# appyjain21/pilottai

Measured on AMD Instinct MI355X. Metric: completed agent-tasks/sec (whole node) + p50 task latency, 64 concurrent workers, higher is better.
Workload: dtype bf16

## Files before the change

### csrc/ops/attention.hip

```cpp
#include "common.h"

#include <algorithm>
#include <cstdlib>

namespace pa {

constexpr int ATT_HD = 128;
constexpr int ATT_BLK = 16;
constexpr int ATT_PART = 512;
constexpr float NEG_BIG = -1.0e30f;

template <int NW>
constexpr int att_lds_decode_bytes() { return (NW * 16 * (ATT_HD + 4) + 2 * NW * 16) * 4; }
constexpr int ATT_LDS_DECODE_BYTES = att_lds_decode_bytes<4>();
typedef __attribute__((address_space(1))) unsigned long long gu64;
typedef __attribute__((address_space(1))) int gi32;

__device__ __forceinline__ void att_store8(bf16* p, const bf16x8 v) { *reinterpret_cast<bf16x8*>(p) = v; }

template <int G, int NW = 4>
__device__ __forceinline__ void decode_item(
    const int4 it, char* smem, bf16* __restrict__ out, float* __restrict__ part_o,
    float* __restrict__ part_ml, int* __restrict__ counters, const bf16* __restrict__ q, const bf16* __restrict__ k_cache,
    const bf16* __restrict__ v_cache, const int* __restrict__ q_start, const int* __restrict__ q_len,
    const int* __restrict__ ctx_len, const int* __restrict__ block_table, int max_blocks, int H,
    int KV, int kvh, float scale_log2, int psz, int acq) {
  const int s = it.x, qb = it.y;
  const int nq = it.z & 0xff, part = (it.z >> 8) & 0xfff, nparts = it.z >> 20;
  const int pidx = it.w;
  const int lane = threadIdx.x & 63, wid = threadIdx.x >> 6;
  const int g = lane >> 4, col = lane & 15;
  const int hg = col % G, tq = col / G;
  const int ctx = ctx_len[s], ql = q_len[s], q0 = q_start[s];

  const bool colvalid = tq < nq;
  const int tok = qb + tq;
  const int key_limit = colvalid ? (ctx - ql + tok + 1) : 0;
  const int head = kvh * G + hg;
  const int causal_end = ctx - ql + qb + nq;
  const int kv_begin = nparts > 1 ? part * psz : 0;
  const int kv_end = nparts > 1 ? min(causal_end, kv_begin + psz) : causal_end;
  const int t_first = kv_begin >> 5;
  const int t_last = (kv_end + 31) >> 5;

  bf16x8 qf[4];
  {
    const bf16* qrow = q + ((size_t)(q0 + (colvalid ? tok : 0)) * H + head) * ATT_HD + 8 * g;
#pragma unroll
    for (int m = 0; m < 4; ++m) {
      bf16x8 v = *reinterpret_cast<const bf16x8*>(qrow + 32 * m);
      if (!colvalid) {
#pragma unroll
        for (int j = 0; j < 8; ++j) v[j] = (bf16)0.f;
      }
      qf[m] = v;
    }
  }

  const int* bt = block_table + (size_t)s * max_blocks;
  const int nblk = (ctx + ATT_BLK - 1) / ATT_BLK;
  const int kin = 8 * (col >> 2) + (col & 3);
  const size_t kv_stride_blk = (size_t)KV * ATT_BLK * ATT_HD;

  f32x4 o[8];
#pragma unroll
  for (int n = 0; n < 8; ++n) o[n] = f32x4{0.f, 0.f, 0.f, 0.f};
  float m_run = NEG_BIG, l_run = 0.f;

  auto load_tile = [&](int t, bf16x8 (&kf)[2][4], bf16x8 (&vf)[8]) {
    const int b0 = min(2 * t, nblk - 1), b1 = min(2 * t + 1, nblk - 1);
    const int pb0 = bt[b0], pb1 = bt[b1];
    const int pk = (kin >= 16) ? pb1 : pb0;
    const bf16* kbase = k_cache + (size_t)pk * kv_stride_blk +
                        (((size_t)kvh * 16 + g) * ATT_BLK + (kin & 15)) * 8;
#pragma unroll
    for (int c = 0; c < 2; ++c)
#pragma unroll
      for (int m = 0; m < 4; ++m)
        kf[c][m] = *reinterpret_cast<const bf16x8*>(kbase + (4 * m * ATT_BLK + 4 * c) * 8);
    const int pv = (g >> 1) ? pb1 : pb0;
    const bf16* vbase =
        v_cache + (size_t)pv * kv_stride_blk + ((size_t)kvh * ATT_HD + col) * ATT_BLK + 8 * (g & 1);
#pragma unroll
    for (int n = 0; n < 8; ++n)
      vf[n] = *reinterpret_cast<const bf16x8*>(vbase + (size_t)16 * n * ATT_BLK);
  };
  bf16x8 kf[2][4], vf[8];
  if (t_first + wid < t_last) load_tile(t_first + wid, kf, vf);
  for (int t = t_first + wid; t < t_last; t += NW) {
    bf16x8 kn[2][4], vn[8];
    if (t + NW < t_last) load_tile(t + NW, kn, vn);

    f32x4 sc[2];
#pragma unroll
    for (int c = 0; c < 2; ++c) {
      f32x4 acc = {0.f, 0.f, 0.f, 0.f};
#pragma unroll
      for (int m = 0; m < 4; ++m)
        acc = __builtin_amdgcn_mfma_f32_16x16x32_bf16(kf[c][m], qf[m], acc, 0, 0, 0);
      sc[c] = acc;
    }
    float tmax = NEG_BIG;
    const int kb = 32 * t + 8 * g;
#pragma unroll
    for (int c = 0; c < 2; ++c)
#pragma unroll
      for (int r = 0; r < 4; ++r) {
        const int key = kb + 4 * c + r;
        float v = sc[c][r] * scale_log2;
        v = (key < key_limit && key >= kv_begin) ? v : NEG_BIG;
        sc[c][r] = v;
        tmax = fmaxf(tmax, v);
      }
    tmax = fmaxf(tmax, __shfl_xor(tmax, 16, 64));
    tmax = fmaxf(tmax, __shfl_xor(tmax, 32, 64));
    const float m_new = fmaxf(m_run, tmax);
    const float alpha = exp2f(m_run - m_new);
    m_run = m_new;
    bf16x8 pf;
    float psum = 0.f;
#pragma unroll
    for (int c = 0; c < 2; ++c)
#pragma unroll
      for (int r = 0; r < 4; ++r) {
        const float p = exp2f(sc[c][r] - m_new);
        psum += p;
        pf[4 * c + r] = (bf16)p;
      }
    l_run = l_run * alpha + psum;
#pragma unroll
    for (int n = 0; n < 8; ++n) {
      o[n] *= alpha;
      o[n] = __builtin_amdgcn_mfma_f32_16x16x32_bf16(vf[n], pf, o[n], 0, 0, 0);
    }
#pragma unroll
    for (int c = 0; c < 2; ++c)
#pragma unroll
      for (int m = 0; m < 4; ++m) kf[c][m] = kn[c][m];
#pragma unroll
    for (int n = 0; n < 8; ++n) vf[n] = vn[n];
  }
  l_run += __shfl_xor(l_run, 16, 64);
  l_run += __shfl_xor(l_run, 32, 64);

  float(*lds_o)[16][ATT_HD + 4] = reinterpret_cast<float(*)[16][ATT_HD + 4]>(smem);
  float(*lds_m)[16] = reinterpret_cast<float(*)[16]>(smem + NW * 16 * (ATT_HD + 4) * sizeof(float));
  float(*lds_l)[16] = lds_m + NW;
#pragma unroll
  for (int n = 0; n < 8; ++n)
#pragma unroll
    for (int r = 0; r < 4; ++r) lds_o[wid][col][16 * n + 4 * g + r] = o[n][r];
  if (g == 0) {
    lds_m[wid][col] = m_run;
    lds_l[wid][col] = l_run;
  }
  __syncthreads();
  const bool mthr = NW == 4 || threadIdx.x < 256;
  const int ccol = (threadIdx.x >> 4) & 15;
  const int d0 = (threadIdx.x & 15) * 8;
  float mt = NEG_BIG;
#pragma unroll
  for (int w = 0; w < NW; ++w) mt = fmaxf(mt, lds_m[w][ccol]);
  float wgt[NW], L = 0.f;
#pragma unroll
  for (int w = 0; w < NW; ++w) {
    wgt[w] = exp2f(lds_m[w][ccol] - mt);
    L += wgt[w] * lds_l[w][ccol];
  }
  float acc[8];
#pragma unroll
  for (int j = 0; j < 8; ++j) {
    float a = 0.f;
#pragma unroll
    for (int w = 0; w < NW; ++w) a += wgt[w] * lds_o[w][ccol][d0 + j];
    acc[j] = a;
  }
  const int ctq = ccol / G, chg = ccol % G;
  if (nparts > 1) {
    const __amdgpu_buffer_rsrc_t ps = __builtin_amdgcn_make_buffer_rsrc(
        part_o + ((size_t)pidx * KV + kvh) * 16 * ATT_HD, 0, 16 * ATT_HD * 4, 0x00020000);
    const int soff = (ccol * ATT_HD + d0) * 4;
    if (mthr) {
      __builtin_amdgcn_raw_buffer_store_b128(__builtin_bit_cast(u32x4, f32x4{acc[0], acc[1], acc[2], acc[3]}),
                                             ps, soff, 0, 16);
      __builtin_amdgcn_raw_buffer_store_b128(__builtin_bit_cast(u32x4, f32x4{acc[4], acc[5], acc[6], acc[7]}),
                                             ps, soff + 16, 0, 16);
    }
    if (mthr && (threadIdx.x & 15) == 0) {
      const unsigned long long mlv =
          ((unsigned long long)__float_as_uint(L) << 32) | (unsigned long long)__float_as_uint(mt);
      __hip_atomic_store((gu64*)(part_ml + (((size_t)pidx * KV + kvh) * 16 + ccol) * 2), mlv,
                         __ATOMIC_RELAXED, __HIP_MEMORY_SCOPE_AGENT);
    }
    int* lflag = reinterpret_cast<int*>(smem + att_lds_decode_bytes<NW>());
    asm volatile("s_waitcnt vmcnt(0)" ::: "memory");
    if (!handoff_last(counters + (size_t)s * KV + kvh, nparts, lflag, acq) || ctq >= nq || !mthr) return;
    const int p0 = pidx - part;
    const __amdgpu_buffer_rsrc_t rs = __builtin_amdgcn_make_buffer_rsrc(
        part_o + (size_t)p0 * KV * 16 * ATT_HD, 0, nparts * KV * 16 * ATT_HD * 4, 0x00020000);
    auto load_ml = [&](int p) {
      return __hip_atomic_load((gu64*)(part_ml + (((size_t)(p0 + p) * KV + kvh) * 16 + ccol) * 2),
                               __ATOMIC_RELAXED, __HIP_MEMORY_SCOPE_AGENT);
    };
    float gm = NEG_BIG;
    for (int p = 0; p < nparts; ++p) gm = fmaxf(gm, __uint_as_float((unsigned)load_ml(p)));
    float GL = 0.f, ga[8] = {0.f, 0.f, 0.f, 0.f, 0.f, 0.f, 0.f, 0.f};
    for (int p = 0; p < nparts; ++p) {
      const unsigned long long v = load_ml(p);
      const float pmv = __uint_as_float((unsigned)v), plv = __uint_as_float((unsigned)(v >> 32));
      const float w = exp2f(pmv - gm);
      GL += w * plv;
      const int roff = (((p * KV + kvh) * 16 + ccol) * ATT_HD + d0) * 4;
      const f32x4 a = __builtin_bit_cast(f32x4, __builtin_amdgcn_raw_buffer_load_b128(rs, roff, 0, 16));
      const f32x4 b = __builtin_bit_cast(f32x4, __builtin_amdgcn_raw_buffer_load_b128(rs, roff + 16, 0, 16));
#pragma unroll
      for (int j = 0; j < 4; ++j) {
        ga[j] += w * a[j];
        ga[4 + j] += w * b[j];
      }
    }
    const float ginv = 1.f / GL;
    bf16x8 g8;
#pragma unroll
    for (int j = 0; j < 8; ++j) g8[j] = (bf16)(ga[j] * ginv);
    att_store8(out + ((size_t)(q0 + qb + ctq) * H + kvh * G + chg) * ATT_HD + d0, g8);
    return;
  }
  if (ctq >= nq || !mthr) return;
  const float inv = 1.f / L;
  bf16x8 w8;
#pragma unroll
  for (int j = 0; j < 8; ++j) w8[j] = (bf16)(acc[j] * inv);
  att_store8(out + ((size_t)(q0 + qb + ctq) * H + kvh * G + chg) * ATT_HD + d0, w8);
}

__device__ __forceinline__ int swap23(int x) { return (x & ~12) | ((x & 4) << 1) | ((x & 8) >> 1); }
constexpr int PF_LD = ATT_HD + 4;

__device__ __forceinline__ void softmax_pv_tile(f32x16 s, bool mask, int key0, int key_limit, float scale_log2,
                                                float& m_run, float& l_run, f32x16 (&o)[4],
                                                const bf16x8 (&vf)[2][4]) {
  if (mask) {
    const int lim = key_limit - key0;
#pragma unroll
    for (int g = 0; g < 16; ++g) s[g] = (16 * (g >> 3) + (g & 7)) < lim ? s[g] : NEG_BIG;
  }
  float tmax = s[0];
#pragma unroll
  for (int g = 1; g < 16; ++g) tmax = fmaxf(tmax, s[g]);
  tmax = fmaxf(tmax, __shfl_xor(tmax, 32, 64));
  const float m_new = fmaxf(m_run, tmax * scale_log2);
  if (__any(m_new > m_run)) {
    const float alpha = __builtin_amdgcn_exp2f(m_run - m_new);
    l_run *= alpha;
#pragma unroll
    for (int m = 0; m < 4; ++m) o[m] *= alpha;
    m_run = m_new;
  }
  const float nm = -m_run;
  float psum = 0.f;
  bf16x8 pf[2];
#pragma unroll
  for (int g = 0; g < 16; ++g) {
    const float p = __builtin_amdgcn_exp2f(fmaf(s[g], scale_log2, nm));
    psum += p;
    pf[g >> 3][g & 7] = (bf16)p;
  }
  l_run += psum;
#pragma unroll
  for (int st = 0; st < 2; ++st)
#pragma unroll
    for (int m = 0; m < 4; ++m) o[m] = __builtin_amdgcn_mfma_f32_32x32x16_bf16(vf[st][m], pf[st], o[m], 0, 0, 0);
}

__device__ __forceinline__ f32x16 qk_tile(const bf16x8 (&kf)[8], const bf16x8 (&qf)[8]) {
  f32x16 s;
#pragma unroll
  for (int j = 0; j < 16; ++j) s[j] = 0.f;
#pragma unroll
  for (int i = 0; i < 8; ++i) s = __builtin_amdgcn_mfma_f32_32x32x16_bf16(kf[i], qf[i], s, 0, 0, 0);
  return s;
}

template <int G, int NW = 4>
__device__ __forceinline__ void prefill_item(
    const int4 it, char* smem, bf16* __restrict__ out, const bf16* __restrict__ q,
    const bf16* __restrict__ k_cache, const bf16* __restrict__ v_cache,
    const int* __restrict__ q_start, const int* __restrict__ q_len, const int* __restrict__ ctx_len,
    const int* __restrict__ block_table, int max_blocks, int H, int KV, int kvh, float scale_log2) {
  const int s = it.x, qb = it.y, nq = it.z & 0xff;
  const int lane = threadIdx.x & 63, wid = threadIdx.x >> 6;
  const int r = lane & 31, h = lane >> 5;
  const int hg = r % G, tq = r / G;
  const int ctx = ctx_len[s], ql = q_len[s], q0 = q_start[s];
  const bool colvalid = tq < nq;
  const int tok = qb + tq;
  const int key_limit = colvalid ? (ctx - ql + tok + 1) : 0;
  const int head = kvh * G + hg;
  const int ntiles = (ctx - ql + qb + nq + 31) >> 5;
  const int kmin = ctx - ql + qb + 1;

  bf16x8 qf[8];
  {
    const bf16* qrow = q + ((size_t)(q0 + (colvalid ? tok : 0)) * H + head) * ATT_HD + 8 * h;
#pragma unroll
    for (int i = 0; i < 8; ++i) {
      bf16x8 v = *reinterpret_cast<const bf16x8*>(qrow + 16 * i);
      if (!colvalid) {
#pragma unroll
        for (int j = 0; j < 8; ++j) v[j] = (bf16)0.f;
      }
      qf[i] = v;
    }
  }
  const int* bt = block_table + (size_t)s * max_blocks;
  const int nblk = (ctx + ATT_BLK - 1) / ATT_BLK;
  const size_t kv_stride_blk = (size_t)KV * ATT_BLK * ATT_HD;
  const int krow = swap23(r);

  f32x16 o[4];
#pragma unroll
  for (int m = 0; m < 4; ++m)
#pragma unroll
    for (int j = 0; j < 16; ++j) o[m][j] = 0.f;
  float m_run = NEG_BIG, l_run = 0.f;

  for (int t = wid; t < ntiles; t += NW) {
    const int pb0 = bt[min(2 * t, nblk - 1)], pb1 = bt[min(2 * t + 1, nblk - 1)];
    const bf16* kbase = k_cache + (size_t)(krow >= 16 ? pb1 : pb0) * kv_stride_blk +
                        (((size_t)kvh * 16 + h) * ATT_BLK + (krow & 15)) * 8;
    bf16x8 kf[8];
#pragma unroll
    for (int i = 0; i < 8; ++i) kf[i] = *reinterpret_cast<const bf16x8*>(kbase + (size_t)2 * i * ATT_BLK * 8);
    bf16x8 vf[2][4];
#pragma unroll
    for (int st = 0; st < 2; ++st) {
      const bf16* vbase = v_cache + (size_t)(st ? pb1 : pb0) * kv_stride_blk +
                          ((size_t)kvh * ATT_HD + r) * ATT_BLK + 8 * h;
#pragma unroll
      for (int m = 0; m < 4; ++m) vf[st][m] = *reinterpret_cast<const bf16x8*>(vbase + (size_t)32 * m * ATT_BLK);
    }
    const f32x16 sc = qk_tile(kf, qf);
    softmax_pv_tile(sc, 32 * t + 32 > kmin, 32 * t + 8 * h, key_limit, scale_log2, m_run, l_run, o, vf);
  }
  l_run += __shfl_xor(l_run, 32, 64);

  float* lo = reinterpret_cast<float*>(smem);
  float* lm = lo + NW * 32 * PF_LD;
  float* ll = lm + NW * 32;
#pragma unroll
  for (int m = 0; m < 4; ++m)
#pragma unroll
    for (int gq = 0; gq < 4; ++gq) {
      f32x4 v = {o[m][4 * gq], o[m][4 * gq + 1], o[m][4 * gq + 2], o[m][4 * gq + 3]};
      *reinterpret_cast<f32x4*>(lo + (wid * 32 + r) * PF_LD + 32 * m + 8 * gq + 4 * h) = v;
    }
  if (h == 0) {
    lm[wid * 32 + r] = m_run;
    ll[wid * 32 + r] = l_run;
  }
  __syncthreads();
  const int ccol = threadIdx.x >> 3, d0 = (threadIdx.x & 7) * 16;
  const int ctq = ccol / G, chg = ccol % G;
  if (ctq >= nq || (NW == 8 && threadIdx.x >= 256)) return;
  float mt = NEG_BIG;
#pragma unroll
  for (int w = 0; w < NW; ++w) mt = fmaxf(mt, lm[w * 32 + ccol]);
  float wgt[NW], L = 0.f;
#pragma unroll
  for (int w = 0; w < NW; ++w) {
    wgt[w] = exp2f(lm[w * 32 + ccol] - mt);
    L += wgt[w] * ll[w * 32 + ccol];
  }
  const float inv = 1.f / L;
  bf16* orow = out + ((size_t)(q0 + qb + ctq) * H + kvh * G + chg) * ATT_HD + d0;
#pragma unroll
  for (int c8 = 0; c8 < 2; ++c8) {
    float acc[8] = {0.f, 0.f, 0.f, 0.f, 0.f, 0.f, 0.f, 0.f};
#pragma unroll
    for (int w = 0; w < NW; ++w) {
      const f32x4* src = reinterpret_cast<const f32x4*>(lo + (w * 32 + ccol) * PF_LD + d0 + 8 * c8);
      const f32x4 a = src[0], b = src[1];
#pragma unroll
      for (int j = 0; j < 4; ++j) {
        acc[j] += wgt[w] * a[j];
        acc[4 + j] += wgt[w] * b[j];
      }
    }
    bf16x8 w8;
#pragma unroll
    for (int j = 0; j < 8; ++j) w8[j] = (bf16)(acc[j] * inv);
    att_store8(orow + 8 * c8, w8);
  }
}

constexpr int PW_TILE = 16384;

typedef __attribute__((address_space(3))) void att_lds_t;
typedef __attribute__((address_space(1))) void att_gbl_t;

constexpr int PW_NBUF = 4;
template <int N>
__device__ __forceinline__ void att_wait_vm() { __builtin_amdgcn_s_waitcnt((N & 15) | ((N >> 4) << 14) | (7 << 4) | (15 << 8)); }

constexpr int PW_PART_SLOTS = 8;

template <int G, bool SPLIT>
__device__ __forceinline__ void prefill_item_wg(
    const int4 it, char* smem, bf16* __restrict__ out, const bf16* __restrict__ q,
    const bf16* __restrict__ k_cache, const bf16* __restrict__ v_cache,
    const int* __restrict__ q_start, const int* __restrict__ q_len, const int* __restrict__ ctx_len,
    const int* __restrict__ block_table, int max_blocks, int H, int KV, int kvh, float scale_log2,
    float* __restrict__ part_o, float* __restrict__ part_ml, int* __restrict__ pf_counters, int acq) {
  constexpr int TPWV = 32 / G;
  const int s = it.x, qb = it.y, nq = it.z & 0xff;
  const int part = SPLIT && pf_counters ? (it.z >> 8) & 0xfff : 0;
  const int nparts = SPLIT && pf_counters ? max(1, it.z >> 20) : 1;
  const int pidx = it.w;
  const int lane = threadIdx.x & 63;
  const int wid = __builtin_amdgcn_readfirstlane(threadIdx.x >> 6);
  const int r = lane & 31, h = lane >> 5;
  const int hg = r % G, tq = wid * TPWV + r / G;
  const int ctx = ctx_len[s], ql = q_len[s], q0 = q_start[s];
  const bool colvalid = tq < nq;
  const int tok = qb + tq;
  const int key_limit = colvalid ? (ctx - ql + tok + 1) : 0;
  const int head = kvh * G + hg;
  const int wave_keys = wid * TPWV < nq ? ctx - ql + qb + min(nq, (wid + 1) * TPWV) : 0;
  const int ntiles_all = (ctx - ql + qb + nq + 31) >> 5;
  const int tpp = (ntiles_all + nparts - 1) / nparts;
  const int t_begin = min(ntiles_all, part * tpp);
  const int ntiles = min(ntiles_all, t_begin + tpp) - t_begin;
  const int kmin = ctx - ql + qb + wid * TPWV + 1;

  bf16x8 qf[8];
  {
    const bf16* qrow = q + ((size_t)(q0 + (colvalid ? tok : 0)) * H + head) * ATT_HD + 8 * h;
#pragma unroll
    for (int i = 0; i < 8; ++i) {
      bf16x8 v = *reinterpret_cast<const bf16x8*>(qrow + 16 * i);
      if (!colvalid) {
#pragma unroll
        for (int j = 0; j < 8; ++j) v[j] = (bf16)0.f;
      }
      qf[i] = v;
    }
  }
  const int* bt = block_table + (size_t)s * max_blocks;
  const int nblk = (ctx + ATT_BLK - 1) / ATT_BLK;
  const size_t kv_stride_blk = (size_t)KV * ATT_BLK * ATT_HD;
  const int krow = swap23(r);
  auto stage = [&](int t, int buf) {
    const int pb0 = bt[min(2 * t, nblk - 1)], pb1 = bt[min(2 * t + 1, nblk - 1)];
#pragma unroll
    for (int i = 0; i < 4; ++i) {
      const int p = wid * 4 + i;
      const int chunk = p < 8 ? lane : lane ^ ((lane >> 4) & 1);
      const bf16* src = (p < 8 ? k_cache : v_cache) + (size_t)(((p >> 2) & 1) ? pb1 : pb0) * kv_stride_blk +
                        (size_t)kvh * ATT_BLK * ATT_HD + (p & 3) * 512 + chunk * 8;
      __builtin_amdgcn_global_load_lds((att_gbl_t*)src, (att_lds_t*)(smem + buf * PW_TILE + p * 1024), 16, 0, 0);
    }
  };

  f32x16 o[4];
#pragma unroll
  for (int m = 0; m < 4; ++m)
#pragma unroll
    for (int j = 0; j < 16; ++j) o[m][j] = 0.f;
  float m_run = NEG_BIG, l_run = 0.f;

#pragma unroll
  for (int p = 0; p < PW_NBUF - 1; ++p)
    if (p < ntiles) stage(t_begin + p, p);
  for (int u = 0; u < ntiles; ++u) {
    const int t = t_begin + u;
    const int buf = u % PW_NBUF;
    const int after = min(PW_NBUF - 2, ntiles - 1 - u);
    if (after >= 2) att_wait_vm<8>();
    else if (after == 1) att_wait_vm<4>();
    else att_wait_vm<0>();
    asm volatile("" ::: "memory");
    __builtin_amdgcn_s_barrier();
    asm volatile("" ::: "memory");
    if (u + PW_NBUF - 1 < ntiles) stage(t + PW_NBUF - 1, (u + PW_NBUF - 1) % PW_NBUF);
    if (32 * t >= wave_keys) continue;
    const char* tb = smem + buf * PW_TILE;
    const char* kb = tb + (krow >= 16 ? 4096 : 0) + ((h * ATT_BLK + (krow & 15)) << 4);
    bf16x8 kf[8];
#pragma unroll
    for (int i = 0; i < 8; ++i) kf[i] = *reinterpret_cast<const bf16x8*>(kb + i * 2 * ATT_BLK * 16);
    bf16x8 vf[2][4];
#pragma unroll
    for (int st = 0; st < 2; ++st)
#pragma unroll
      for (int m = 0; m < 4; ++m)
        vf[st][m] = *reinterpret_cast<const bf16x8*>(tb + 8192 + st * 4096 + (32 * m + r) * 32 +
                                                     16 * (h ^ ((r >> 3) & 1)));
    const f32x16 sc = qk_tile(kf, qf);
    softmax_pv_tile(sc, 32 * t + 32 > kmin, 32 * t + 8 * h, key_limit, scale_log2, m_run, l_run, o, vf);
  }
  l_run += __shfl_xor(l_run, 32, 64);
  if (SPLIT && nparts > 1) {
    const int p0 = pidx - PW_PART_SLOTS * part;
    auto chunk = [&](int slot0, int j) { return part_o + ((size_t)(slot0 + j) * KV + kvh) * 16 * ATT_HD; };
#pragma unroll
    for (int m = 0; m < 4; ++m) {
      const __amdgpu_buffer_rsrc_t ps = __builtin_amdgcn_make_buffer_rsrc(chunk(pidx, 2 * wid + (m >> 1)), 0,
                                                                          16 * ATT_HD * 4, 0x00020000);
#pragma unroll
      for (int c4 = 0; c4 < 4; ++c4)
        __builtin_amdgcn_raw_buffer_store_b128(
            __builtin_bit_cast(u32x4, f32x4{o[m][4 * c4], o[m][4 * c4 + 1], o[m][4 * c4 + 2], o[m][4 * c4 + 3]}), ps,
            ((((m & 1) * 64 + lane) * 16) + 4 * c4) * 4, 0, 16);
    }
    const int pcol = 32 * wid + r;
    if (h == 0) {
      const unsigned long long mlv =
          ((unsigned long long)__float_as_uint(l_run) << 32) | (unsigned long long)__float_as_uint(m_run);
      __hip_atomic_store((gu64*)(part_ml + ((size_t)(pidx + pcol / 16) * KV + kvh) * 32 + (pcol % 16) * 2), mlv,
                         __ATOMIC_RELAXED, __HIP_MEMORY_SCOPE_AGENT);
    }
    int* lflag = reinterpret_cast<int*>(smem + PW_NBUF * PW_TILE);
    asm volatile("s_waitcnt vmcnt(0)" ::: "memory");
    if (!handoff_last(pf_counters + (size_t)p0 * KV + kvh, nparts, lflag, acq)) return;
    float gm = NEG_BIG;
    for (int p = 0; p < nparts; ++p) {
      const unsigned long long v = __hip_atomic_load(
          (gu64*)(part_ml + ((size_t)(p0 + PW_PART_SLOTS * p + pcol / 16) * KV + kvh) * 32 + (pcol % 16) * 2),
          __ATOMIC_RELAXED, __HIP_MEMORY_SCOPE_AGENT);
      gm = fmaxf(gm, __uint_as_float((unsigned)v));
    }
    float GL = 0.f;
#pragma unroll
    for (int m = 0; m < 4; ++m) o[m] = f32x16{};
    for (int p = 0; p < nparts; ++p) {
      const int sp = p0 + PW_PART_SLOTS * p;
      const unsigned long long v = __hip_atomic_load(
          (gu64*)(part_ml + ((size_t)(sp + pcol / 16) * KV + kvh) * 32 + (pcol % 16) * 2), __ATOMIC_RELAXED,
          __HIP_MEMORY_SCOPE_AGENT);
      const float w = __builtin_amdgcn_exp2f(__uint_as_float((unsigned)v) - gm);
      GL += w * __uint_as_float((unsigned)(v >> 32));
#pragma unroll
      for (int m = 0; m < 4; ++m) {
        const __amdgpu_buffer_rsrc_t rs = __builtin_amdgcn_make_buffer_rsrc(chunk(sp, 2 * wid + (m >> 1)), 0,
                                                                            16 * ATT_HD * 4, 0x00020000);
#pragma unroll
        for (int c4 = 0; c4 < 4; ++c4) {
          const f32x4 a = __builtin_bit_cast(
              f32x4, __builtin_amdgcn_raw_buffer_load_b128(rs, ((((m & 1) * 64 + lane) * 16) + 4 * c4) * 4, 0, 16));
#pragma unroll
          for (int e = 0; e < 4; ++e) o[m][4 * c4 + e] += w * a[e];
        }
      }
    }
    l_run = GL;
  }
  const float inv = l_run > 0.f ? 1.f / l_run : 0.f;

  __syncthreads();
  char* img = smem + wid * 8192;
#pragma unroll
  for (int m = 0; m < 4; ++m)
#pragma unroll
    for (int gq = 0; gq < 4; ++gq) {
      bf16x4 v;
#pragma unroll
      for (int j = 0; j < 4; ++j) v[j] = (bf16)(o[m][4 * gq + j] * inv);
      *reinterpret_cast<bf16x4*>(img + (r * ATT_HD + 32 * m + 8 * gq + 4 * h) * 2) = v;
    }
  __syncthreads();
  const int ccol = lane >> 1, dhalf = (lane & 1) * 64;
  const int ctq = wid * TPWV + ccol / G, chg = ccol % G;
  if (ctq < nq) {
    bf16* orow = out + ((size_t)(q0 + qb + ctq) * H + kvh * G + chg) * ATT_HD + dhalf;
#pragma unroll
    for (int c8 = 0; c8 < 8; ++c8)
      *reinterpret_cast<bf16x8*>(orow + 8 * c8) =
          *reinterpret_cast<const bf16x8*>(img + (ccol * ATT_HD + dhalf + 8 * c8) * 2);
  }
}

template <int G, int NW, bool SPLIT>
__device__ __forceinline__ void prefill_any(
    const int4 it, char* smem, bf16* __restrict__ out, const bf16* __restrict__ q,
    const bf16* __restrict__ k_cache, const bf16* __restrict__ v_cache,
    const int* __restrict__ q_start, const int* __restrict__ q_len, const int* __restrict__ ctx_len,
    const int* __restrict__ block_table, int max_blocks, int H, int KV, int kvh, float scale_log2,
    float* __restrict__ part_o, float* __restrict__ part_ml, int* __restrict__ pf_counters, int acq) {
  const int nq = it.z & 0xff;
  if (nq <= 32 / G) {
    prefill_item<G, NW>(it, smem, out, q, k_cache, v_cache, q_start, q_len, ctx_len, block_table, max_blocks,
                            H, KV, kvh, scale_log2);
  } else if constexpr (NW == 4) {
    prefill_item_wg<G, SPLIT>(it, smem, out, q, k_cache, v_cache, q_start, q_len, ctx_len, block_table, max_blocks, H, KV,
                       kvh, scale_log2, part_o, part_ml, pf_counters, acq);
  } else {
    for (int sb = 0; sb < nq; sb += 32 / G) {
      const int4 sub = {it.x, it.y + sb, min(32 / G, nq - sb) | (it.z & ~0xff), it.w};
      prefill_item<G, NW>(sub, smem, out, q, k_cache, v_cache, q_start, q_len, ctx_len, block_table,
                              max_blocks, H, KV, kvh, scale_log2);
      __syncthreads();
    }
  }
}

constexpr int ATT_LDS_DECODE = ATT_LDS_DECODE_BYTES + 16;
constexpr int ATT_LDS_BYTES8 = std::max(att_lds_decode_bytes<8>() + 16, (8 * 32 * PF_LD + 2 * 8 * 32) * 4);
constexpr int ATT_LDS_PREFILL = (4 * 32 * PF_LD + 2 * 4 * 32) * 4;
constexpr int ATT_LDS_BYTES0 = ATT_LDS_PREFILL > ATT_LDS_DECODE ? ATT_LDS_PREFILL : ATT_LDS_DECODE;
constexpr int ATT_LDS_BYTES0W = ATT_LDS_BYTES0 > PW_NBUF * PW_TILE + 16 ? ATT_LDS_BYTES0 : PW_NBUF * PW_TILE + 16;
constexpr int ATT_LDS_BYTES = ATT_LDS_BYTES0W;

template <int G, int NW = 4, bool SPLIT = false>
__global__ __launch_bounds__(64 * NW, NW == 4 ? 2 : 1) void paged_attn_kernel(
    bf16* __restrict__ out, float* __restrict__ part_o, float* __restrict__ part_ml,
    int* __restrict__ counters, const bf16* __restrict__ q, const bf16* __restrict__ k_cache,
    const bf16* __restrict__ v_cache, const int4* __restrict__ items,
    const int* __restrict__ n_items, const int* __restrict__ part_size, const int* __restrict__ q_start,
    const int* __restrict__ q_len, const int* __restrict__ ctx_len,
    const int* __restrict__ block_table, int max_blocks, int H, int KV, float scale_log2, int acq,
    int* __restrict__ pf_counters) {
  extern __shared__ __attribute__((aligned(16))) char smem[];
  constexpr int TPW = 16 / G;
  const int psz_q = part_size ? part_size[0] : ATT_PART;
  const int kvh = blockIdx.x;
  const int slot = blockIdx.y;
  const int nslots = gridDim.y;
  const int n = n_items[0];
  int4 it_next = items[min(slot, max(n - 1, 0))];
  if (slot >= n) return;
  const int psz = psz_q;
  for (int item = slot; item < n; item += nslots) {
    const int4 it = it_next;
    if (item + nslots < n) it_next = items[item + nslots];
    const int nq = it.z & 0xff;
    if (nq <= TPW)
      decode_item<G, NW>(it, smem, out, part_o, part_ml, counters, q, k_cache, v_cache, q_start, q_len, ctx_len,
                         block_table, max_blocks, H, KV, kvh, scale_log2, psz, acq);
    else
      prefill_any<G, NW, SPLIT>(it, smem, out, q, k_cache, v_cache, q_start, q_len, ctx_len, block_table, max_blocks, H,
                         KV, kvh, scale_log2, part_o, part_ml, pf_counters, acq);
    __syncthreads();
  }
}

}

extern "C" int pa_paged_attention(void* out, float* part_o, float* part_ml, const void* q,
                                  const void* k_cache, const void* v_cache, const int* items,
                                  const int* n_items, int max_items, const int* part_size, int* counters,
                                  const int* q_start, const int* q_len, const int* ctx_len, const int* block_table,
                                  int max_blocks, int H, int KV, float scale_log2, int waves, int* pf_counters,
                                  hipStream_t st) {
  if (H % KV != 0) return -1;
  if (waves != 4 && waves != 8) return -1;
  const int G = H / KV;
  const int gx = max_items < 1 ? 1 : (max_items < 2048 / KV ? max_items : (2048 / KV > 0 ? 2048 / KV : 1));
  const dim3 grid(KV, gx);
#define PA_ATT(GG)                                                                              \
  do {                                                                                          \
    if (max_items <= 0) break;                                                                  \
    if (waves == 8) {                                                                           \
      static bool attr8 = false;                                                                \
      if (!attr8) {                                                                             \
        (void)hipFuncSetAttribute((const void*)pa::paged_attn_kernel<GG, 8>,                    \
                                  hipFuncAttributeMaxDynamicSharedMemorySize, pa::ATT_LDS_BYTES8); \
        attr8 = true;                                                                           \
      }                                                                                         \
      hipLaunchKernelGGL((pa::paged_attn_kernel<GG, 8>), grid, dim3(512), pa::ATT_LDS_BYTES8, st, \
                         (pa::bf16*)out, part_o, part_ml, counters, (const pa::bf16*)q,         \
                         (const pa::bf16*)k_cache, (const pa::bf16*)v_cache, (const int4*)items, \
                         n_items, part_size, q_start, q_len, ctx_len, block_table, max_blocks, H, \
                         KV, scale_log2, pa::g_handoff_attn, pf_counters);                      \
      break;                                                                                    \
    }                                                                                           \
    static bool attr4 = false;                                                                  \
    if (!attr4) {                                                                               \
      (void)hipFuncSetAttribute((const void*)pa::paged_attn_kernel<GG, 4, false>,               \
                                hipFuncAttributeMaxDynamicSharedMemorySize, pa::ATT_LDS_BYTES); \
      (void)hipFuncSetAttribute((const void*)pa::paged_attn_kernel<GG, 4, true>,                \
                                hipFuncAttributeMaxDynamicSharedMemorySize, pa::ATT_LDS_BYTES); \
      attr4 = true;                                                                             \
    }                                                                                           \
    if (pf_counters)          \
      hipLaunchKernelGGL((pa::paged_attn_kernel<GG, 4, true>), grid, dim3(256), pa::ATT_LDS_BYTES, st, \
                         (pa::bf16*)out, part_o, part_ml, counters, (const pa::bf16*)q,         \
                         (const pa::bf16*)k_cache, (const pa::bf16*)v_cache, (const int4*)items, \
                         n_items, part_size, q_start, q_len, ctx_len, block_table, max_blocks, H, \
                         KV, scale_log2, pa::g_handoff_attn, pf_counters);                      \
    else                                                                                        \
      hipLaunchKernelGGL((pa::paged_attn_kernel<GG, 4, false>), grid, dim3(256), pa::ATT_LDS_BYTES, st, \
                         (pa::bf16*)out, part_o, part_ml, counters, (const pa::bf16*)q,         \
                         (const pa::bf16*)k_cache, (const pa::bf16*)v_cache, (const int4*)items, \
                         n_items, part_size, q_start, q_len, ctx_len, block_table, max_blocks, H, \
                         KV, scale_log2, pa::g_handoff_attn, nullptr);                          \
  } while (0)
  switch (G) {
    case 1: PA_ATT(1); break;
    case 2: PA_ATT(2); break;
    case 4: PA_ATT(4); break;
    case 8: PA_ATT(8); break;
    case 16: PA_ATT(16); break;
    default: return -2;
  }
#undef PA_ATT
  return (int)hipGetLastError();
}
```

Baseline: 42.94.

## Batch scalar metadata loads and prefetch block-table ids ahead of KV tile loads

Sequence lengths and the first block-table entries are now fetched with one batched inline-asm s_load group and a single wait, instead of dependent vector loads. Block ids for later tiles are prefetched one iteration ahead through constant-address-space scalar loads, so each KV tile load no longer waits on a block-table load. This applies to the decode, prefill and pipelined prefill paths, and the wave id is made uniform with readfirstlane. The aim is to cut per-item setup latency and the pointer-chasing stall in the tile loop. The cost is more complex code, early reads that rely on clamping against max_blocks, and hand-written asm that depends on the exact operand layout.

After: 43.27 (median of 4 runs). No clear change (+0.8%).

```diff
diff --git a/csrc/ops/attention.hip b/csrc/ops/attention.hip
--- a/csrc/ops/attention.hip
+++ b/csrc/ops/attention.hip
@@ -17,6 +17,53 @@
 typedef __attribute__((address_space(1))) int gi32;
 
 __device__ __forceinline__ void att_store8(bf16* p, const bf16x8 v) { *reinterpret_cast<bf16x8*>(p) = v; }
+
+struct seq_lens { int ctx, ql, q0; };
+__device__ __forceinline__ seq_lens item_loads(const int* cl, const int* qlp, const int* qs, const int* bt,
+                                               const int (&o)[2], int (&e)[2]) {
+  seq_lens r;
+  asm volatile(
+      "s_load_dword %0, %5, 0x0\n s_load_dword %1, %6, 0x0\n s_load_dword %2, %7, 0x0\n"
+      "s_load_dword %3, %8, %9\n s_load_dword %4, %8, %10\n s_waitcnt lgkmcnt(0)"
+      : "=&s"(r.ctx), "=&s"(r.ql), "=&s"(r.q0), "=&s"(e[0]), "=&s"(e[1])
+      : "s"(cl), "s"(qlp), "s"(qs), "s"(bt), "s"(o[0]), "s"(o[1]));
+  return r;
+}
+__device__ __forceinline__ seq_lens item_loads(const int* cl, const int* qlp, const int* qs, const int* bt,
+                                               const int (&o)[4], int (&e)[4]) {
+  seq_lens r;
+  asm volatile(
+      "s_load_dword %0, %7, 0x0\n s_load_dword %1, %8, 0x0\n s_load_dword %2, %9, 0x0\n"
+      "s_load_dword %3, %10, %11\n s_load_dword %4, %10, %12\n s_load_dword %5, %10, %13\n"
+      "s_load_dword %6, %10, %14\n s_waitcnt lgkmcnt(0)"
+      : "=&s"(r.ctx), "=&s"(r.ql), "=&s"(r.q0), "=&s"(e[0]), "=&s"(e[1]), "=&s"(e[2]), "=&s"(e[3])
+      : "s"(cl), "s"(qlp), "s"(qs), "s"(bt), "s"(o[0]), "s"(o[1]), "s"(o[2]), "s"(o[3]));
+  return r;
+}
+__device__ __forceinline__ seq_lens item_loads(const int* cl, const int* qlp, const int* qs, const int* bt,
+                                               const int (&o)[8], int (&e)[8]) {
+  seq_lens r;
+  asm volatile(
+      "s_load_dword %0, %11, 0x0\n s_load_dword %1, %12, 0x0\n s_load_dword %2, %13, 0x0\n"
+      "s_load_dword %3, %14, %15\n s_load_dword %4, %14, %16\n s_load_dword %5, %14, %17\n"
+      "s_load_dword %6, %14, %18\n s_load_dword %7, %14, %19\n s_load_dword %8, %14, %20\n"
+      "s_load_dword %9, %14, %21\n s_load_dword %10, %14, %22\n s_waitcnt lgkmcnt(0)"
+      : "=&s"(r.ctx), "=&s"(r.ql), "=&s"(r.q0), "=&s"(e[0]), "=&s"(e[1]), "=&s"(e[2]), "=&s"(e[3]), "=&s"(e[4]),
+        "=&s"(e[5]), "=&s"(e[6]), "=&s"(e[7])
+      : "s"(cl), "s"(qlp), "s"(qs), "s"(bt), "s"(o[0]), "s"(o[1]), "s"(o[2]), "s"(o[3]), "s"(o[4]), "s"(o[5]),
+        "s"(o[6]), "s"(o[7]));
+  return r;
+}
+
+typedef __attribute__((address_space(4))) const int att_cint;
+__device__ __forceinline__ int2 bt_fetch(const int* bt, int t, int nblk) {
+  att_cint* cb = (att_cint*)(unsigned long long)bt;
+  return int2{cb[min(2 * t, nblk - 1)], cb[min(2 * t + 1, nblk - 1)]};
+}
+__device__ __forceinline__ int bt_early(int blk, int max_blocks) { return 4 * min(blk, max_blocks - 1); }
+__device__ __forceinline__ int2 bt_ids(int2 e, int t, int nblk) {
+  return int2{e.x, 2 * t + 1 < nblk ? e.y : e.x};
+}
 
 template <int G, int NW = 4>
 __device__ __forceinline__ void decode_item(
@@ -28,19 +75,27 @@
   const int s = it.x, qb = it.y;
   const int nq = it.z & 0xff, part = (it.z >> 8) & 0xfff, nparts = it.z >> 20;
   const int pidx = it.w;
-  const int lane = threadIdx.x & 63, wid = threadIdx.x >> 6;
+  const int lane = threadIdx.x & 63;
+  const int wid = __builtin_amdgcn_readfirstlane(threadIdx.x >> 6);
   const int g = lane >> 4, col = lane & 15;
   const int hg = col % G, tq = col / G;
-  const int ctx = ctx_len[s], ql = q_len[s], q0 = q_start[s];
+  const int* bt = block_table + (size_t)s * max_blocks;
+  const int kv_begin = nparts > 1 ? part * psz : 0;
+  const int t_first = kv_begin >> 5;
+  const int tw = t_first + wid;
+  const int eo[4] = {bt_early(2 * tw, max_blocks), bt_early(2 * tw + 1, max_blocks),
+                     bt_early(2 * (tw + NW), max_blocks), bt_early(2 * (tw + NW) + 1, max_blocks)};
+  int ev[4];
+  const seq_lens sl = item_loads(ctx_len + s, q_len + s, q_start + s, bt, eo, ev);
+  const int ctx = sl.ctx, ql = sl.ql, q0 = sl.q0;
+  const int2 e0 = {ev[0], ev[1]}, e1 = {ev[2], ev[3]};
 
   const bool colvalid = tq < nq;
   const int tok = qb + tq;
   const int key_limit = colvalid ? (ctx - ql + tok + 1) : 0;
   const int head = kvh * G + hg;
   const int causal_end = ctx - ql + qb + nq;
-  const int kv_begin = nparts > 1 ? part * psz : 0;
   const int kv_end = nparts > 1 ? min(causal_end, kv_begin + psz) : causal_end;
-  const int t_first = kv_begin >> 5;
   const int t_last = (kv_end + 31) >> 5;
 
   bf16x8 qf[4];
@@ -57,7 +112,6 @@
     }
   }
 
-  const int* bt = block_table + (size_t)s * max_blocks;
   const int nblk = (ctx + ATT_BLK - 1) / ATT_BLK;
   const int kin = 8 * (col >> 2) + (col & 3);
   const size_t kv_stride_blk = (size_t)KV * ATT_BLK * ATT_HD;
@@ -67,9 +121,8 @@
   for (int n = 0; n < 8; ++n) o[n] = f32x4{0.f, 0.f, 0.f, 0.f};
   float m_run = NEG_BIG, l_run = 0.f;
 
-  auto load_tile = [&](int t, bf16x8 (&kf)[2][4], bf16x8 (&vf)[8]) {
-    const int b0 = min(2 * t, nblk - 1), b1 = min(2 * t + 1, nblk - 1);
-    const int pb0 = bt[b0], pb1 = bt[b1];
+  auto load_tile = [&](const int2 pb, bf16x8 (&kf)[2][4], bf16x8 (&vf)[8]) {
+    const int pb0 = pb.x, pb1 = pb.y;
     const int pk = (kin >= 16) ? pb1 : pb0;
     const bf16* kbase = k_cache + (size_t)pk * kv_stride_blk +
                         (((size_t)kvh * 16 + g) * ATT_BLK + (kin & 15)) * 8;
@@ -85,12 +138,7 @@
     for (int n = 0; n < 8; ++n)
       vf[n] = *reinterpret_cast<const bf16x8*>(vbase + (size_t)16 * n * ATT_BLK);
   };
-  bf16x8 kf[2][4], vf[8];
-  if (t_first + wid < t_last) load_tile(t_first + wid, kf, vf);
-  for (int t = t_first + wid; t < t_last; t += NW) {
-    bf16x8 kn[2][4], vn[8];
-    if (t + NW < t_last) load_tile(t + NW, kn, vn);
-
+  auto tile = [&](int t, const bf16x8 (&kf)[2][4], const bf16x8 (&vf)[8]) {
     f32x4 sc[2];
 #pragma unroll
     for (int c = 0; c < 2; ++c) {
@@ -133,12 +181,25 @@
       o[n] *= alpha;
       o[n] = __builtin_amdgcn_mfma_f32_16x16x32_bf16(vf[n], pf, o[n], 0, 0, 0);
     }
-#pragma unroll
-    for (int c = 0; c < 2; ++c)
-#pragma unroll
-      for (int m = 0; m < 4; ++m) kf[c][m] = kn[c][m];
-#pragma unroll
-    for (int n = 0; n < 8; ++n) vf[n] = vn[n];
+  };
+  int t = t_first + wid;
+  if (t < t_last) {
+    bf16x8 kf[2][4], vf[8];
+    load_tile(bt_ids(e0, t, nblk), kf, vf);
+    int2 cur = bt_ids(e1, t + NW, nblk);
+    for (; t + NW < t_last; t += NW) {
+      bf16x8 kn[2][4], vn[8];
+      load_tile(cur, kn, vn);
+      if (t + 2 * NW < t_last) cur = bt_fetch(bt, t + 2 * NW, nblk);
+      tile(t, kf, vf);
+#pragma unroll
+      for (int c = 0; c < 2; ++c)
+#pragma unroll
+        for (int m = 0; m < 4; ++m) kf[c][m] = kn[c][m];
+#pragma unroll
+      for (int n = 0; n < 8; ++n) vf[n] = vn[n];
+    }
+    tile(t, kf, vf);
   }
   l_run += __shfl_xor(l_run, 16, 64);
   l_run += __shfl_xor(l_run, 32, 64);
@@ -289,10 +350,16 @@
     const int* __restrict__ q_start, const int* __restrict__ q_len, const int* __restrict__ ctx_len,
     const int* __restrict__ block_table, int max_blocks, int H, int KV, int kvh, float scale_log2) {
   const int s = it.x, qb = it.y, nq = it.z & 0xff;
-  const int lane = threadIdx.x & 63, wid = threadIdx.x >> 6;
+  const int lane = threadIdx.x & 63;
+  const int wid = __builtin_amdgcn_readfirstlane(threadIdx.x >> 6);
   const int r = lane & 31, h = lane >> 5;
   const int hg = r % G, tq = r / G;
-  const int ctx = ctx_len[s], ql = q_len[s], q0 = q_start[s];
+  const int* bt = block_table + (size_t)s * max_blocks;
+  const int eo[2] = {bt_early(2 * wid, max_blocks), bt_early(2 * wid + 1, max_blocks)};
+  int ev[2];
+  const seq_lens sl = item_loads(ctx_len + s, q_len + s, q_start + s, bt, eo, ev);
+  const int ctx = sl.ctx, ql = sl.ql, q0 = sl.q0;
+  const int2 e0 = {ev[0], ev[1]};
   const bool colvalid = tq < nq;
   const int tok = qb + tq;
   const int key_limit = colvalid ? (ctx - ql + tok + 1) : 0;
@@ -313,7 +380,6 @@
       qf[i] = v;
     }
   }
-  const int* bt = block_table + (size_t)s * max_blocks;
   const int nblk = (ctx + ATT_BLK - 1) / ATT_BLK;
   const size_t kv_stride_blk = (size_t)KV * ATT_BLK * ATT_HD;
   const int krow = swap23(r);
@@ -325,8 +391,9 @@
     for (int j = 0; j < 16; ++j) o[m][j] = 0.f;
   float m_run = NEG_BIG, l_run = 0.f;
 
+  int2 cur = bt_ids(e0, wid, nblk);
   for (int t = wid; t < ntiles; t += NW) {
-    const int pb0 = bt[min(2 * t, nblk - 1)], pb1 = bt[min(2 * t + 1, nblk - 1)];
+    const int pb0 = cur.x, pb1 = cur.y;
     const bf16* kbase = k_cache + (size_t)(krow >= 16 ? pb1 : pb0) * kv_stride_blk +
                         (((size_t)kvh * 16 + h) * ATT_BLK + (krow & 15)) * 8;
     bf16x8 kf[8];
@@ -340,6 +407,7 @@
 #pragma unroll
       for (int m = 0; m < 4; ++m) vf[st][m] = *reinterpret_cast<const bf16x8*>(vbase + (size_t)32 * m * ATT_BLK);
     }
+    if (t + NW < ntiles) cur = bt_fetch(bt, t + NW, nblk);
     const f32x16 sc = qk_tile(kf, qf);
     softmax_pv_tile(sc, 32 * t + 32 > kmin, 32 * t + 8 * h, key_limit, scale_log2, m_run, l_run, o, vf);
   }
@@ -421,7 +489,16 @@
   const int wid = __builtin_amdgcn_readfirstlane(threadIdx.x >> 6);
   const int r = lane & 31, h = lane >> 5;
   const int hg = r % G, tq = wid * TPWV + r / G;
-  const int ctx = ctx_len[s], ql = q_len[s], q0 = q_start[s];
+  const int* bt = block_table + (size_t)s * max_blocks;
+  static_assert(PW_NBUF == 4, "item_loads fetches the ids of four tiles");
+  int eo[8], ev[8];
+#pragma unroll
+  for (int b = 0; b < 8; ++b) eo[b] = bt_early(b, max_blocks);
+  const seq_lens sl = item_loads(ctx_len + s, q_len + s, q_start + s, bt, eo, ev);
+  const int ctx = sl.ctx, ql = sl.ql, q0 = sl.q0;
+  int2 ids[PW_NBUF];
+#pragma unroll
+  for (int p = 0; p < PW_NBUF; ++p) ids[p] = int2{ev[2 * p], ev[2 * p + 1]};
   const bool colvalid = tq < nq;
   const int tok = qb + tq;
   const int key_limit = colvalid ? (ctx - ql + tok + 1) : 0;
@@ -446,12 +523,18 @@
       qf[i] = v;
     }
   }
-  const int* bt = block_table + (size_t)s * max_blocks;
   const int nblk = (ctx + ATT_BLK - 1) / ATT_BLK;
   const size_t kv_stride_blk = (size_t)KV * ATT_BLK * ATT_HD;
   const int krow = swap23(r);
-  auto stage = [&](int t, int buf) {
-    const int pb0 = bt[min(2 * t, nblk - 1)], pb1 = bt[min(2 * t + 1, nblk - 1)];
+  if (SPLIT && t_begin > 0) {
+#pragma unroll
+    for (int p = 0; p < PW_NBUF; ++p) ids[p] = bt_fetch(bt, t_begin + p, nblk);
+  } else {
+#pragma unroll
+    for (int p = 0; p < PW_NBUF; ++p) ids[p] = bt_ids(ids[p], p, nblk);
+  }
+  auto stage = [&](const int2 pb, int buf) {
+    const int pb0 = pb.x, pb1 = pb.y;
 #pragma unroll
     for (int i = 0; i < 4; ++i) {
       const int p = wid * 4 + i;
@@ -471,7 +554,8 @@
 
 #pragma unroll
   for (int p = 0; p < PW_NBUF - 1; ++p)
-    if (p < ntiles) stage(t_begin + p, p);
+    if (p < ntiles) stage(ids[p], p);
+  int2 cur = ids[PW_NBUF - 1];
   for (int u = 0; u < ntiles; ++u) {
     const int t = t_begin + u;
     const int buf = u % PW_NBUF;
@@ -482,7 +566,8 @@
     asm volatile("" ::: "memory");
     __builtin_amdgcn_s_barrier();
     asm volatile("" ::: "memory");
-    if (u + PW_NBUF - 1 < ntiles) stage(t + PW_NBUF - 1, (u + PW_NBUF - 1) % PW_NBUF);
+    if (u + PW_NBUF - 1 < ntiles) stage(cur, (u + PW_NBUF - 1) % PW_NBUF);
+    if (u + PW_NBUF < ntiles) cur = bt_fetch(bt, t + PW_NBUF, nblk);
     if (32 * t >= wave_keys) continue;
     const char* tb = smem + buf * PW_TILE;
     const char* kb = tb + (krow >= 16 ? 4096 : 0) + ((h * ATT_BLK + (krow & 15)) << 4);
```
